# wolfi/NeuroSync_Trainer_Lite

Hardware: AMD Instinct MI355X
Metric: train frames/sec (audio->blendshape) 228M cfg (higher is better)
Workload: dtype bf16

## Files before the change

neurosync_trainer_lite_amd/csrc/gemm4.h:

```cpp
#pragma once
#include "common.h"
#include <type_traits>

namespace g4 {

constexpr int NT = 256;
constexpr int TILE = 256;
constexpr int BK = 64;
constexpr int OPS = 32768;
constexpr int SMEM = 4 * OPS;
constexpr int ROPE_LDS = 32768;
constexpr int GROUP_MAX = 16;

enum { EM_BF16 = 1, EM_RELU_DROP = 2, EM_ROPE = 3, EM_DRELU = 4, EM_F32 = 5 };

struct Params {
  const char* A; int64_t lda;
  const char* B; int64_t ldb;
  char* C; int64_t ldc;
  int M, N, K;
  float alpha;
  const float* bias;
  float inv_keep; uint32_t thresh; uint64_t seed;
  const float* rope_cos; const float* rope_sin; int rope_T, rope_dim, rope_cols;
  float* colsum_part;
  uint64_t* relu_mask;
  float* sq_part;
  const float* a_scale;
  const float* b_scale;
  int rope_bf16;
  uint32_t a_bytes, b_bytes;
  int tiles_m, tiles_n;
};

struct StreamK {
  float* slab;
  unsigned* cnt;
  uint32_t slab_bytes;
  int dp_tiles;
  int units;
};

struct GroupParams {
  Params g[GROUP_MAX];
  int tile_end[GROUP_MAX];
  int n;
  StreamK sk;
};
static_assert(sizeof(GroupParams) <= 4096, "kernel arguments");

typedef int i32x4_t __attribute__((ext_vector_type(4)));
typedef int i32x2_t __attribute__((ext_vector_type(2)));
typedef __attribute__((address_space(3))) void lds_void_t;

NSTL_DEV uint32_t lds_addr(const char* p) { return (uint32_t)(uintptr_t)(const __attribute__((address_space(3))) char*)p; }

#define G4_VMCNT(n) asm volatile("s_waitcnt vmcnt(" #n ")" ::: "memory")
#define G4_SB() __builtin_amdgcn_sched_barrier(0)
#define G4_LGKM0()                                      \
  do {                                                  \
    asm volatile("s_waitcnt lgkmcnt(0)" ::: "memory"); \
    G4_SB();                                            \
  } while (0)

NSTL_DEV void dma16(__amdgpu_buffer_rsrc_t r, char* lds, uint32_t voff, uint32_t soff) {
  __builtin_amdgcn_raw_ptr_buffer_load_lds(r, (lds_void_t*)lds, 16, voff, soff, 0, 0);
}

constexpr int SIDE_W = 2048;
constexpr int SIDE_LDS = 4 * SIDE_W;

template <bool KMAJ>
NSTL_DEV void dma_lane_offsets(uint32_t (&vo)[8], int64_t ld, int wave, int lane) {
#pragma unroll
  for (int s = 0; s < 8; ++s) {
    const int q = wave * 8 + s;
    if (KMAJ) {
      const int row = 8 * q + (lane >> 3), pc = lane & 7;
      const int lc = pc ^ ((row >> 1) & 7);
      vo[s] = (uint32_t)(((int64_t)row * ld + lc * 8) * 2);
    } else {
      const int row = 2 * q + (lane >> 5), pc = lane & 31;
// ... 118 lines not shown
                        char* bdst, uint32_t sa, uint32_t sb) {
  if constexpr (I < 64) {
    if constexpr (!(DBG & 8)) {
      if constexpr (Z) mma16z(acc[I >> 3][I & 7], cb[I & 7], ca[I >> 3]);
      else mma16(acc[I >> 3][I & 7], cb[I & 7], ca[I >> 3]);
    }
    G4_SB();
    if constexpr (RD && !(DBG & 2))
      rd_after<AK, BKM, RSOA, RSOB, RH, I, 0, (DBG & 256) ? 56 : (DBG & 512) ? 32 : (DBG & 1024) ? 24 : 46>(na, nb, ra,
                                                                                                       rb);
    if constexpr ((DMAM == 2 || DMAM == 3) && !(DBG & 1) && (I & 7) == ((DBG & 2048) ? 6 : 2)) {
      constexpr int q = I >> 3;
      if constexpr (DMAM == 2) dma16(d.ra, adst + q * 1024, d.va[q], d.ta + sa);
      else dma16(d.rb, bdst + q * 1024, d.vb[q], d.tb + sb);
      G4_SB();
    }
    constexpr bool DMA_HERE = (DBG & 16)    ? I < 16
                              : (DBG & 32)  ? (I < 32 && (I & 1) == 0)
                              : (DBG & 64)  ? (I >= 32 && (I & 1) == 0)
                              : (DBG & 128) ? (I >= 47 && I < 63)
                                            : (I & 3) == 2;
    if constexpr (DMAM == 1 && !(DBG & 1) && DMA_HERE) {
      constexpr int q = (DBG & 16)    ? I
                        : (DBG & 32)  ? I >> 1
                        : (DBG & 64)  ? (I - 32) >> 1
                        : (DBG & 128) ? I - 47
                                      : I >> 2;
      if constexpr (q < 8) dma16(d.ra, adst + q * 1024, d.va[q], d.ta + sa);
      else dma16(d.rb, bdst + (q - 8) * 1024, d.vb[q - 8], d.tb + sb);
      G4_SB();
    }
    half_step<AK, BKM, RD, RSOA, RSOB, RH, DMAM, DBG, Z, I + 1>(acc, ca, cb, na, nb, ra, rb, d, adst, bdst, sa, sb);
  }
}

NSTL_DEV void tile_coords(int id, int nt_m, int nt_n, int& m0, int& n0) {
  constexpr int GROUP_M = 4;
  const int per_group = GROUP_M * nt_n;
  const int first_m = (id / per_group) * GROUP_M;
  const int gm = min(nt_m - first_m, GROUP_M);
  const int in_g = id % per_group;
  m0 = (first_m + in_g % gm) * TILE;
  n0 = (in_g / gm) * TILE;
}

typedef float f32x2_t __attribute__((ext_vector_type(2)));
typedef __bf16 bf16x2_t __attribute__((ext_vector_type(2)));
NSTL_DEV uint32_t pack_bf16x2(float lo, float hi) {
  return __builtin_bit_cast(uint32_t, __builtin_convertvector((f32x2_t){lo, hi}, bf16x2_t));
}
NSTL_DEV float bf16_lo(uint32_t w) { return __uint_as_float(w << 16); }
NSTL_DEV float bf16_hi(uint32_t w) { return __uint_as_float(w & 0xFFFF0000u); }
NSTL_DEV uint32_t asr31(uint32_t x) {
  uint32_t r;
  asm("v_ashrrev_i32 %0, 31, %1" : "=v"(r) : "v"(x));
  return r;
}
NSTL_DEV uint32_t min1(uint32_t x) {
  uint32_t r;
  asm("v_min_u32 %0, 1, %1" : "=v"(r) : "v"(x));
  return r;
}
NSTL_DEV uint32_t keep_lo_mask(uint32_t h, uint32_t thresh) { return asr31(thresh - 1u - (h & 0xFFFFu)); }
NSTL_DEV uint32_t keep_hi_mask(uint32_t h, uint32_t thresh) { return asr31(thresh - 1u - (h >> 16)); }
NSTL_DEV float and_mask(float x, uint32_t m) { return __uint_as_float(__float_as_uint(x) & m); }
NSTL_DEV uint32_t pos_bits2(uint32_t w) {
// ... 58 lines not shown
  float r0, r1, r2, r3;
  if constexpr (ZW == 2) {
    asm volatile(
        "v_accvgpr_read_b32 %0, %4\n\t"
        "v_accvgpr_read_b32 %1, %5\n\t"
        "v_accvgpr_read_b32 %2, %6\n\t"
        "v_accvgpr_read_b32 %3, %7"
        : "=&v"(r0), "=&v"(r1), "=&v"(r2), "=&v"(r3)
        : "a"(x[0]), "a"(x[1]), "a"(x[2]), "a"(x[3]));
    asm volatile("v_mfma_f32_16x16x16_bf16 %0, %1, %1, 0" : "+a"(x) : "v"(z));
  } else if constexpr (ZW == 1) {
    asm volatile(
        "v_accvgpr_read_b32 %0, %4\n\t"
        "v_accvgpr_read_b32 %1, %5\n\t"
        "v_accvgpr_read_b32 %2, %6\n\t"
        "v_accvgpr_read_b32 %3, %7\n\t"
        "v_accvgpr_write_b32 %4, 0\n\t"
        "v_accvgpr_write_b32 %5, 0\n\t"
        "v_accvgpr_write_b32 %6, 0\n\t"
        "v_accvgpr_write_b32 %7, 0"
        : "=&v"(r0), "=&v"(r1), "=&v"(r2), "=&v"(r3), "+a"(x[0]), "+a"(x[1]), "+a"(x[2]), "+a"(x[3]));
  } else {
    asm volatile(
        "v_accvgpr_read_b32 %0, %4\n\t"
        "v_accvgpr_read_b32 %1, %5\n\t"
        "v_accvgpr_read_b32 %2, %6\n\t"
        "v_accvgpr_read_b32 %3, %7"
        : "=&v"(r0), "=&v"(r1), "=&v"(r2), "=&v"(r3)
        : "a"(x[0]), "a"(x[1]), "a"(x[2]), "a"(x[3]));
  }
  return (f32x4){r0, r1, r2, r3};
}

NSTL_DEV f32x4 rd_acc_keep(const f32x4& x) {
  float r0, r1, r2, r3;
  asm volatile(
      "v_accvgpr_read_b32 %0, %4\n\t"
      "v_accvgpr_read_b32 %1, %5\n\t"
      "v_accvgpr_read_b32 %2, %6\n\t"
      "v_accvgpr_read_b32 %3, %7"
      : "=&v"(r0), "=&v"(r1), "=&v"(r2), "=&v"(r3)
      : "a"(x[0]), "a"(x[1]), "a"(x[2]), "a"(x[3]));
  return (f32x4){r0, r1, r2, r3};
}
NSTL_DEV void add_acc(f32x4& x, const f32x4 y) {
  float t0, t1, t2, t3;
  asm volatile(
      "v_accvgpr_read_b32 %0, %4\n\t"
      "v_accvgpr_read_b32 %1, %5\n\t"
      "v_accvgpr_read_b32 %2, %6\n\t"
      "v_accvgpr_read_b32 %3, %7\n\t"
      "v_add_f32 %0, %0, %8\n\t"
      "v_add_f32 %1, %1, %9\n\t"
      "v_add_f32 %2, %2, %10\n\t"
      "v_add_f32 %3, %3, %11\n\t"
      "v_accvgpr_write_b32 %4, %0\n\t"
      "v_accvgpr_write_b32 %5, %1\n\t"
      "v_accvgpr_write_b32 %6, %2\n\t"
      "v_accvgpr_write_b32 %7, %3"
      : "=&v"(t0), "=&v"(t1), "=&v"(t2), "=&v"(t3), "+a"(x[0]), "+a"(x[1]), "+a"(x[2]), "+a"(x[3])
      : "v"(y[0]), "v"(y[1]), "v"(y[2]), "v"(y[3]));
}

struct Seg {
  int t, ks, ke;
};
struct Walker {
  int t_dp, G, dp_tiles, U;
  int rank;
  int pos, end;
  NSTL_DEV void init(const GroupParams& gp, int T, int w, int G_, bool sk) {
    G = G_;
    t_dp = w;
    rank = w;
    if (sk) {
      dp_tiles = gp.sk.dp_tiles;
      U = gp.sk.units;
      if (G % 8 == 0) rank = xcd_remap(w, G);
      const int I = (T - dp_tiles) * U;
      pos = rank * I / G;
      end = (rank + 1) * I / G;
    } else {
      dp_tiles = T;
      U = 1;
      pos = end = 0;
    }
  }
  NSTL_DEV bool next(Seg& s) {
    if (t_dp < dp_tiles) {
      s.t = t_dp;
      s.ks = 0;
      s.ke = -1;
      t_dp += G;
      return true;
    }
    if (pos >= end) return false;
    s.t = dp_tiles + pos / U;
    s.ks = pos % U;
    s.ke = s.ks + end - pos < U ? s.ks + end - pos : U;
    pos += s.ke - s.ks;
    return true;
  }
};

NSTL_DEV bool sk_handoff(const StreamK& sk, f32x4 (&acc)[8][8], const Seg& s, int w, int wave, int lane) {
  const bool part = !(s.ke < 0 || (s.ks == 0 && s.ke == sk.units));
  const bool tail = s.ks > 0;
  const uint32_t mine = (uint32_t)(tail ? 2 * w : 2 * w + 1), other = (uint32_t)(tail ? 2 * w - 1 : 2 * w + 2);
  const __amdgpu_buffer_rsrc_t r =
      __builtin_amdgcn_make_buffer_rsrc((void*)sk.slab, 0, part ? (int)sk.slab_bytes : 0, 0x00020000);
// ... 265 lines not shown
          uint32_t lo = (uint32_t)w, hi = (uint32_t)(w >> 32);
          lo |= (uint32_t)__builtin_amdgcn_mov_dpp((int)lo, 0x128, 0xF, 0xF, false);
          hi |= (uint32_t)__builtin_amdgcn_mov_dpp((int)hi, 0x128, 0xF, 0xF, false);
          const auto slo = __builtin_amdgcn_permlane16_swap(lo, lo, false, false);
          const auto shi = __builtin_amdgcn_permlane16_swap(hi, hi, false, false);
          lo = slo[0] | slo[1];
          hi = shi[0] | shi[1];
          if (fin && c < 8 && odd == 0)
            p.relu_mask[mask_word(p.N, row0 + 64 * hb + c, col0 + 16 * b + 4 * g)] = ((uint64_t)hi << 32) | lo;
        }
    }
    if (EM == EM_DRELU && p.colsum_part != nullptr) {
#pragma unroll
      for (int b = 0; b < 8; ++b)
#pragma unroll
        for (int e = 0; e < 4; ++e) {
          float x = csum[b][e];
          x += NSTL_DPP(x, 0xB1);
          x += NSTL_DPP(x, 0x4E);
          x += NSTL_DPP(x, 0x141);
          x += NSTL_DPP(x, 0x140);
          csum[b][e] = x;
        }
      if (fin && c == 0) {
        float* dst = p.colsum_part + (int64_t)(row0 >> 7) * p.N + col0 + 4 * g;
#pragma unroll
        for (int b = 0; b < 8; ++b) *(f32x4*)(dst + 16 * b) = (f32x4){csum[b][0], csum[b][1], csum[b][2], csum[b][3]};
      }
    }
  }
}

template <bool AK, bool BKM, int EM, bool GROUPED, int DBG = 0, bool SK = false, int R3 = 0>
__global__ __launch_bounds__(NT, 1) void gemm4_kernel(const GroupParams gp) {
  constexpr bool A3 = R3 == 1, B3 = R3 == 2;
  static_assert(!(R3 && EM == EM_ROPE), "the 3 + 2 ring fills the LDS: no room for the RoPE table");
  constexpr bool SIDE = !R3 && (EM == EM_BF16 || (EM == EM_RELU_DROP && BKM) || EM == EM_DRELU) && !(DBG & 16384);
  constexpr int SMEM_ALL = R3 ? 5 * OPS : SMEM + (EM == EM_ROPE ? ROPE_LDS : 0) + (SIDE ? SIDE_LDS : 0);
  constexpr int B_BASE = A3 ? 3 * OPS : 2 * OPS;
  constexpr bool ZC = !BKM && !SK;
  __shared__ __attribute__((aligned(16))) char smem[SMEM_ALL];
  const int tid = threadIdx.x, lane = tid & 63;
  const int wave = __builtin_amdgcn_readfirstlane(tid >> 6);
  const int wm = wave >> 1, wn = wave & 1;
  const int T = gp.tile_end[gp.n - 1];
  const int G = gridDim.x;
  Walker wk;
  wk.init(gp, T, blockIdx.x, G, SK);
  Seg sg;
  if (!wk.next(sg)) return;
  const uint32_t smem_u32 = lds_addr(smem);
  char* const adst0 = smem + wave * 8 * 1024;
  char* const bdst0 = smem + B_BASE + wave * 8 * 1024;
  const char* rope_lds = smem + SMEM;
  char* const side = smem + SMEM + wave * SIDE_W;
  if constexpr (EM == EM_ROPE) {
    const Params& p0 = gp.g[0];
    const int half = p0.rope_dim >> 1, chunks = p0.rope_dim >> 2, swz = rope_swz(p0.rope_dim);
    for (int i = tid; i < p0.rope_T * chunks; i += NT) {
      const int tt = i / chunks, k = i - tt * chunks;
      const float2 cs = *(const float2*)(p0.rope_cos + tt * half + 2 * k);
      const float2 sn = *(const float2*)(p0.rope_sin + tt * half + 2 * k);
      *(f32x4*)(smem + SMEM + rope_off(tt, k, p0.rope_dim * 4, swz)) = (f32x4){cs.x, sn.x, cs.y, sn.y};
    }
    __syncthreads();
  }

  const int ndp_all = SK ? gp.sk.dp_tiles : T;
  auto locate = [&](int tt, int& prob, int& m0, int& n0, int& lt) {
    const int gt = tt < ndp_all ? xcd_remap(tt, ndp_all) : tt;
    prob = 0;
    if (GROUPED)
      while (prob + 1 < gp.n && gt >= gp.tile_end[prob]) ++prob;
    const int first = prob ? gp.tile_end[prob - 1] : 0;
    const Params& q = gp.g[prob];
    lt = gt - first;
    tile_coords(lt, q.tiles_m, q.tiles_n, m0, n0);
  };
  int prob, m0, n0, lt;
  locate(sg.t, prob, m0, n0, lt);
  Dma d;
  dma_lanes<AK, BKM>(d, gp.g[prob], wave, lane);
  dma_tile<AK, BKM>(d, gp.g[prob], m0, n0, sg.ks);
  RdAddr<AK> ra;
  RdAddr<BKM> rb;
  rd_addr<AK>(ra, smem_u32, wm * 128, lane);
  rd_addr<BKM>(rb, smem_u32 + B_BASE, wn * 128, lane);

  f32x4 acc[8][8];
#pragma unroll
  for (int a = 0; a < 8; ++a)
#pragma unroll
    for (int b = 0; b < 8; ++b) acc[a][b] = (f32x4){0.f, 0.f, 0.f, 0.f};
  bf16x8 f0a[8], f0b[8], f1a[8], f1b[8];
#pragma unroll
  for (int s = 0; s < 2; ++s) {
#pragma unroll
    for (int q = 0; q < 8; ++q) dma16(d.ra, adst0 + s * OPS + q * 1024, d.va[q], d.ta + (uint32_t)s * d.a_kb);
#pragma unroll
    for (int q = 0; q < 8; ++q) dma16(d.rb, bdst0 + s * OPS + q * 1024, d.vb[q], d.tb + (uint32_t)s * d.b_kb);
  }
  G4_VMCNT(0);
  __builtin_amdgcn_s_barrier();
  G4_SB();
  rd_all<AK, BKM, 0>(f0a, f0b, ra, rb);
  G4_LGKM0();

  int s3_cur = 0;
  auto move3 = [&](int from, int to) {
    const uint32_t delta = (uint32_t)((to - from) * OPS);
    if constexpr (A3) {
      if constexpr (AK) {
#pragma unroll
        for (int h = 0; h < 2; ++h) ra.k[h] += delta;
      } else {
#pragma unroll
        for (int j = 0; j < 8; ++j) ra.t[j] += delta;
      }
    } else if constexpr (B3) {
      if constexpr (BKM) {
#pragma unroll
        for (int h = 0; h < 2; ++h) rb.k[h] += delta;
      } else {
#pragma unroll
        for (int j = 0; j < 8; ++j) rb.t[j] += delta;
      }
    }
  };

  auto step = [&](auto slot_c, auto waitn_c, uint32_t dma_stage, const Dma& dd) {
    constexpr int S = decltype(slot_c)::value;
    constexpr int WAITN = decltype(waitn_c)::value;
    if constexpr (R3 && WAITN != 0 && !(DBG & 4096)) {
      const int s3_dma = s3_cur == 0 ? 2 : s3_cur - 1;
      const int s3_next = s3_cur == 2 ? 0 : s3_cur + 1;
      const uint32_t oa = dma_stage * dd.a_kb, ob = dma_stage * dd.b_kb;
      half_step<AK, BKM, true, A3 ? 0 : S * OPS, B3 ? 0 : S * OPS, 1, 0, DBG, ZC>(acc, f0a, f0b, f1a, f1b, ra, rb,
                                                                               dd, adst0, bdst0, 0, 0);
      G4_LGKM0();
      if constexpr (WAITN == 32) G4_VMCNT(32);
      else G4_VMCNT(63);
      __builtin_amdgcn_s_barrier();
      G4_SB();
      move3(s3_cur, s3_next);
      half_step<AK, BKM, true, A3 ? 0 : (1 - S) * OPS, B3 ? 0 : (1 - S) * OPS, 0, 1, DBG>(
          acc, f1a, f1b, f0a, f0b, ra, rb, dd, adst0 + (A3 ? s3_dma : S) * OPS, bdst0 + (B3 ? s3_dma : S) * OPS, oa,
          ob);
      G4_LGKM0();
      s3_cur = s3_next;
    } else if constexpr (R3) {
      const int s3_dma = s3_cur == 0 ? 2 : s3_cur - 1;
      const int s3_next = s3_cur == 2 ? 0 : s3_cur + 1;
      const uint32_t oa = dma_stage * dd.a_kb, ob = dma_stage * dd.b_kb;
      half_step<AK, BKM, true, A3 ? 0 : S * OPS, B3 ? 0 : S * OPS, 1, A3 ? 2 : 3, DBG, ZC && WAITN != 0>(
          acc, f0a, f0b, f1a, f1b, ra, rb, dd, adst0 + s3_dma * OPS, bdst0 + s3_dma * OPS, oa, ob);
      G4_LGKM0();
      if constexpr (WAITN == 0) G4_VMCNT(8);
      else if constexpr (WAITN == 32) G4_VMCNT(40);
      else G4_VMCNT(63);
      __builtin_amdgcn_s_barrier();
      G4_SB();
      move3(s3_cur, s3_next);
      half_step<AK, BKM, true, A3 ? 0 : (1 - S) * OPS, B3 ? 0 : (1 - S) * OPS, 0, A3 ? 3 : 2, DBG>(
          acc, f1a, f1b, f0a, f0b, ra, rb, dd, adst0 + S * OPS, bdst0 + S * OPS, oa, ob);
      G4_LGKM0();
      s3_cur = s3_next;
    } else {
      half_step<AK, BKM, true, S * OPS, S * OPS, 1, 0, DBG, ZC && WAITN != 0>(acc, f0a, f0b, f1a, f1b, ra, rb, dd,
                                                                              adst0, bdst0, 0, 0);
      G4_LGKM0();
      if constexpr (WAITN == 0) G4_VMCNT(0);
      else if constexpr (WAITN == 32) G4_VMCNT(32);
      else G4_VMCNT(63);
      __builtin_amdgcn_s_barrier();
      G4_SB();
      half_step<AK, BKM, true, (1 - S) * OPS, (1 - S) * OPS, 0, 1, DBG>(acc, f1a, f1b, f0a, f0b, ra, rb, dd,
                                                                      adst0 + S * OPS, bdst0 + S * OPS,
                                                                      dma_stage * dd.a_kb, dma_stage * dd.b_kb);
      G4_LGKM0();
    }
  };
  using S0 = std::integral_constant<int, 0>;
  using S1 = std::integral_constant<int, 1>;
  using W0 = std::integral_constant<int, 0>;
  using WE = std::integral_constant<int, EM == EM_F32 ? 63 : 32>;

  for (;;) {
    const Params& p = gp.g[prob];
    const int nk = sg.ke < 0 ? p.K / BK : 4 * (sg.ke - sg.ks);
    Seg ns;
    const bool has_next = wk.next(ns);
    if (!has_next) ns = sg;
    int nprob = prob, nm0 = m0, nn0 = n0, nlt = lt;
    if (has_next) locate(ns.t, nprob, nm0, nn0, nlt);
    if constexpr (SIDE) side_dma<EM>(p, side, m0 + wm * 128, n0 + wn * 128, lane);
    step(S0{}, WE{}, 2u, d);
    for (int kt = 1; kt < nk; kt += 2) {
      step(S1{}, W0{}, (uint32_t)(kt + 2 < nk ? kt + 2 : kt + 2 - nk), d);
      if (kt + 1 < nk) {
        if (kt + 1 == nk - 2) {
          if (GROUPED && nprob != prob) dma_lanes<AK, BKM>(d, gp.g[nprob], wave, lane);
          dma_tile<AK, BKM>(d, gp.g[nprob], nm0, nn0, ns.ks, has_next || (DBG & 32768));
        }
        step(S0{}, W0{}, (uint32_t)(kt + 3 < nk ? kt + 3 : kt + 3 - nk), d);
      }
    }
    bool fin = true;
    if constexpr (SK) fin = sk_handoff(gp.sk, acc, sg, wk.rank, wave, lane);
    epilogue<EM, false, (DBG & 8192) ? 1 : 0, ZC ? 0 : (SK ? 1 : 2), SIDE>(p, acc, m0 + wm * 128, n0 + wn * 128, lane,
                                                                        wave, lt, rope_lds, fin, side);
    if (!has_next) break;
    sg = ns;
    prob = nprob;
    m0 = nm0;
    n0 = nn0;
    lt = nlt;
  }
  G4_VMCNT(0);
}

constexpr int F8_BK = 128;

typedef int i32x8_t __attribute__((ext_vector_type(8)));

NSTL_DEV void mma_f8(f32x4& acc, const i32x8_t& w, const i32x8_t& x) {
  acc = __builtin_amdgcn_mfma_scale_f32_16x16x128_f8f6f4(w, x, acc, 0, 0, 0, 0x7f7f7f7f, 0, 0x7f7f7f7f);
}
NSTL_DEV void mma_f8z(f32x4& acc, const i32x8_t& w, const i32x8_t& x) {
  acc = __builtin_amdgcn_mfma_scale_f32_16x16x128_f8f6f4(w, x, (f32x4){0.f, 0.f, 0.f, 0.f}, 0, 0, 0, 0x7f7f7f7f, 0,
                                                          0x7f7f7f7f);
}

NSTL_DEV void dma_lane_offsets_f8(uint32_t (&vo)[8], int64_t ld, int wave, int lane) {
#pragma unroll
  for (int s = 0; s < 8; ++s) {
    const int q = wave * 8 + s;
    const int row = 8 * q + (lane >> 3), pc = lane & 7;
    const int lc = pc ^ ((row >> 1) & 7);
    vo[s] = (uint32_t)((int64_t)row * ld + lc * 16);
  }
}
NSTL_DEV void dma_tile_f8(Dma& d, const Params& p, int m0, int n0, bool live = true) {
  d.ra = __builtin_amdgcn_make_buffer_rsrc((void*)p.A, 0, live ? (int)p.a_bytes : 0, 0x00020000);
  d.rb = __builtin_amdgcn_make_buffer_rsrc((void*)p.B, 0, live ? (int)p.b_bytes : 0, 0x00020000);
  d.a_kb = F8_BK;
  d.b_kb = F8_BK;
  d.ta = __builtin_amdgcn_readfirstlane((uint32_t)(m0 * p.lda));
  d.tb = __builtin_amdgcn_readfirstlane((uint32_t)(n0 * p.ldb));
}

struct RdAddrF8 {
// ... 23 lines not shown
      G4_SB();
    }
    if constexpr (!(DBG & 8)) {
      if constexpr (Z) mma_f8z(acc[4 * (H ? 1 : 0) + a][b], cb[b], ca[a]);
      else mma_f8(acc[4 * (H ? 1 : 0) + a][b], cb[b], ca[a]);
    }
    G4_SB();
    if constexpr (!(DBG & 2)) {
      if constexpr (H == 0 && (I == 1 || I == 6 || I == 11 || I == 16)) {
        constexpr int r = I == 1 ? 0 : I == 6 ? 1 : I == 11 ? 2 : 3;
        rd_f8<SO + (4 + r) * 2048>(na[r], ra);
        G4_SB();
      }
      if constexpr (H == 1 && (I & 7) == 0) {
        rd_f8<SO + (I >> 3) * 2048>(na[I >> 3], ra);
        G4_SB();
      }
      if constexpr (H == 1 && a == 3) {
        rd_f8<SO + b * 2048>(cb[b], rb);
        G4_SB();
      }
    }
    if constexpr (H >= 1 && !(DBG & 1) && (I & 1) == 1) {
      constexpr int q = I >> 1;
      if constexpr (q < 8) dma16(d.ra, adst + q * 1024, d.va[q], d.ta + sa);
      else dma16(d.rb, bdst + (q - 8) * 1024, d.vb[q - 8], d.tb + sb);
      G4_SB();
    }
    half_step_f8<H, SO, DBG, Z, I + 1>(acc, ca, cb, na, ra, rb, d, adst, bdst, sa, sb);
  }
}

template <int EM, int DBG = 0>
__global__ __launch_bounds__(NT, 1) void gemm4f8_kernel(const GroupParams gp) {
  constexpr bool SIDE = EM != EM_ROPE && EM != EM_F32 && !(DBG & 16384);
  __shared__ __attribute__((aligned(16))) char smem[SMEM + (EM == EM_ROPE ? ROPE_LDS : 0) + (SIDE ? 4 * SIDE_W_SC : 0)];
  const int tid = threadIdx.x, lane = tid & 63;
  const int wave = __builtin_amdgcn_readfirstlane(tid >> 6);
  const int wm = wave >> 1, wn = wave & 1;
  const int T = gp.tile_end[0];
  const int G = gridDim.x;
  const Params& p = gp.g[0];
  Walker wk;
  wk.init(gp, T, blockIdx.x, G, false);
  Seg sg;
  if (!wk.next(sg)) return;
  const uint32_t smem_u32 = lds_addr(smem);
  char* const adst0 = smem + wave * 8 * 1024;
  char* const bdst0 = smem + 2 * OPS + wave * 8 * 1024;
  const char* rope_lds = smem + SMEM;
  char* const side = smem + SMEM + wave * SIDE_W_SC;
  if constexpr (EM == EM_ROPE) {
    const int half = p.rope_dim >> 1, chunks = p.rope_dim >> 2, swz = rope_swz(p.rope_dim);
    for (int i = tid; i < p.rope_T * chunks; i += NT) {
      const int tt = i / chunks, k = i - tt * chunks;
      const float2 cs = *(const float2*)(p.rope_cos + tt * half + 2 * k);
      const float2 sn = *(const float2*)(p.rope_sin + tt * half + 2 * k);
      if (p.rope_bf16) {
        *(uint2*)(smem + SMEM + rope_off8(tt, k, p.rope_dim * 2, swz)) =
            make_uint2(pack_bf16x2(cs.x, sn.x), pack_bf16x2(cs.y, sn.y));
      } else {
        *(f32x4*)(smem + SMEM + rope_off(tt, k, p.rope_dim * 4, swz)) = (f32x4){cs.x, sn.x, cs.y, sn.y};
      }
    }
    __syncthreads();
  }
  int m0, n0;
  tile_coords(xcd_remap(sg.t, T), p.tiles_m, p.tiles_n, m0, n0);
  int lt = 0;
  Dma d;
  dma_lane_offsets_f8(d.va, p.lda, wave, lane);
  dma_lane_offsets_f8(d.vb, p.ldb, wave, lane);
  dma_tile_f8(d, p, m0, n0);
  RdAddrF8 ra, rb;
  rd_addr_f8(ra, smem_u32, wm * 128, lane);
  rd_addr_f8(rb, smem_u32 + 2 * OPS, wn * 128, lane);

// ... 80 lines not shown
```

neurosync_trainer_lite_amd/csrc/gemm4.hip:

```cpp
#include <stdlib.h>
#include <string.h>

#include <map>
#include <mutex>
#include <vector>

#include "../../include/nstl.h"
#include "common.h"
#include "gemm4.h"
#include "status.h"

namespace {

int gemm4_env() {
  const char* e = getenv("NSTL_GEMM4");
  return e ? atoi(e) : 1;
}

int sk_env() {
  const char* e = getenv("NSTL_GEMM4_SK");
  return e ? atoi(e) : 0;
}

struct SkSpace {
  float* slab = nullptr;
  unsigned* cnt = nullptr;
  int G = 0;
};
constexpr size_t SK_SPACES = 4;
bool sk_space(hipStream_t st, int G, g4::StreamK& sk) {
  static std::mutex mu;
  static std::map<std::pair<int, hipStream_t>, SkSpace> spaces;
  static std::vector<SkSpace> retired;
  const int dev = nstl::stream_device(st);
  std::lock_guard<std::mutex> lk(mu);
  if (spaces.find({dev, st}) == spaces.end() && spaces.size() >= SK_SPACES) return false;
  SkSpace& s = spaces[{dev, st}];
  if (s.G < G) {
    nstl::DeviceGuard on(dev);
    hipStreamCaptureStatus cs = hipStreamCaptureStatusNone;
    if (hipStreamIsCapturing(st, &cs) != hipSuccess || cs != hipStreamCaptureStatusNone) return false;
    if (s.slab) retired.push_back(s);
    s = SkSpace();
    if (hipMalloc((void**)&s.slab, (size_t)2 * G * 262144) != hipSuccess) return false;
    if (hipMalloc((void**)&s.cnt, (size_t)8 * G * sizeof(unsigned)) != hipSuccess) return false;
    if (hipMemset(s.cnt, 0, (size_t)8 * G * sizeof(unsigned)) != hipSuccess) return false;
    s.G = G;
  }
  sk.slab = s.slab;
  sk.cnt = s.cnt;
  sk.slab_bytes = (uint32_t)((size_t)2 * G * 262144);
  return true;
}

void plan_sk(g4::GroupParams& gp, int G, hipStream_t st) {
  memset(&gp.sk, 0, sizeof(gp.sk));
  const int T = gp.tile_end[gp.n - 1];
  const int mode = sk_env();
  if (T < G || !mode || (T % G == 0 && mode != 2)) return;
  const int K = gp.g[0].K;
  for (int i = 0; i < gp.n; ++i)
    if (gp.g[i].K != K) return;
  if (K % (4 * g4::BK)) return;
  g4::StreamK sk;
  if (!sk_space(st, G, sk)) {
    (void)hipGetLastError();
    return;
  }
  sk.dp_tiles = (T / G - 1) * G;
  sk.units = K / (4 * g4::BK);
  gp.sk = sk;
}

int g4_mode(const nstl_gemm_args* a) {
  if (a->dtype != NSTL_BF16 || a->split_k > 1 || a->beta != 0.f || (a->sq_part != nullptr && a->c_dtype != NSTL_F32))
    return 0;
  const bool bf_out = a->c_dtype == NSTL_BF16;
  if (a->colsum_part != nullptr && a->epilogue != NSTL_EPI_DRELU_DROP) return 0;
  if (a->relu_mask != nullptr && a->epilogue != NSTL_EPI_BIAS_RELU_DROP && a->epilogue != NSTL_EPI_DRELU_DROP)
    return 0;
  switch (a->epilogue) {
    case NSTL_EPI_NONE:
      return bf_out ? g4::EM_BF16 : g4::EM_F32;
    case NSTL_EPI_BIAS:
      return bf_out ? g4::EM_BF16 : 0;
    case NSTL_EPI_BIAS_RELU_DROP:
      return bf_out && (a->N & 1) == 0 ? g4::EM_RELU_DROP : 0;
    case NSTL_EPI_BIAS_ROPE:
      return bf_out && a->b_kmajor && a->rope_dim % 4 == 0 && a->rope_cols % 16 == 0 &&
// ... 19 lines not shown
  return ae < (1ll << 31) && be < (1ll << 31) && ce < (1ll << 31);
}

void fill(g4::Params& q, const nstl_gemm_args* a) {
  memset(&q, 0, sizeof(q));
  q.A = (const char*)a->A; q.lda = a->lda;
  q.B = (const char*)a->B; q.ldb = a->ldb;
  q.C = (char*)a->C; q.ldc = a->ldc;
  q.M = a->M; q.N = a->N; q.K = a->K;
  q.alpha = a->alpha;
  q.bias = a->bias;
  q.thresh = nstl_drop_thresh(a->p_drop);
  q.inv_keep = 1.0f / (1.0f - a->p_drop);
  q.seed = a->seed;
  q.rope_cos = a->rope_cos; q.rope_sin = a->rope_sin;
  q.rope_T = a->rope_T; q.rope_dim = a->rope_dim; q.rope_cols = a->rope_cols;
  q.colsum_part = a->colsum_part;
  q.relu_mask = a->relu_mask;
  q.sq_part = a->sq_part;
  q.a_bytes = (uint32_t)(a->a_kmajor ? ((int64_t)(a->M - 1) * a->lda + a->K) * 2 : ((int64_t)(a->K - 1) * a->lda + a->M) * 2);
  q.b_bytes = (uint32_t)(a->b_kmajor ? ((int64_t)(a->N - 1) * a->ldb + a->K) * 2 : ((int64_t)(a->K - 1) * a->ldb + a->N) * 2);
  q.tiles_m = a->M / g4::TILE;
  q.tiles_n = a->N / g4::TILE;
}

int r3_env() {
  const char* e = getenv("NSTL_GEMM4_R3");
  return e ? atoi(e) : 1;
}

template <bool AK, bool BKM, bool GROUPED, bool SK, int R3>
void launch_em(int em, dim3 grid, hipStream_t st, const g4::GroupParams& gp) {
  const dim3 block(g4::NT);
  switch (em) {
    case g4::EM_BF16: hipLaunchKernelGGL((g4::gemm4_kernel<AK, BKM, g4::EM_BF16, GROUPED, 0, SK, R3>), grid, block, 0, st, gp); break;
    case g4::EM_RELU_DROP:
      hipLaunchKernelGGL((g4::gemm4_kernel<AK, BKM, g4::EM_RELU_DROP, GROUPED, 0, SK, R3>), grid, block, 0, st, gp);
      break;
    case g4::EM_ROPE:
      if constexpr (BKM && !R3) hipLaunchKernelGGL((g4::gemm4_kernel<AK, BKM, g4::EM_ROPE, GROUPED, 0, SK>), grid, block, 0, st, gp);
      break;
    case g4::EM_DRELU: hipLaunchKernelGGL((g4::gemm4_kernel<AK, BKM, g4::EM_DRELU, GROUPED, 0, SK, R3>), grid, block, 0, st, gp); break;
    default: hipLaunchKernelGGL((g4::gemm4_kernel<AK, BKM, g4::EM_F32, GROUPED, 0, SK, R3>), grid, block, 0, st, gp); break;
  }
}

template <bool SK, int R3>
int launch_sk(int em, bool ak, bool bk, bool grouped, dim3 grid, hipStream_t st, const g4::GroupParams& gp) {
  if (ak && bk) {
    if (grouped) {
      if (em != g4::EM_ROPE || SK || R3) return 0;
      hipLaunchKernelGGL((g4::gemm4_kernel<true, true, g4::EM_ROPE, true, 0, false, 0>), grid, dim3(g4::NT), 0, st, gp);
      return 1;
    }
    launch_em<true, true, false, SK, R3>(em, grid, st, gp);
  } else if (ak && !bk) {
    if (grouped) return 0;
    launch_em<true, false, false, SK, R3>(em, grid, st, gp);
  } else {
    if (em != g4::EM_F32) return 0;
    if (grouped) hipLaunchKernelGGL((g4::gemm4_kernel<false, false, g4::EM_F32, true, 0, SK, R3>), grid, dim3(g4::NT), 0, st, gp);
    else hipLaunchKernelGGL((g4::gemm4_kernel<false, false, g4::EM_F32, false, 0, SK, R3>), grid, dim3(g4::NT), 0, st, gp);
  }
  return 1;
}

int launch(int em, bool ak, bool bk, bool grouped, int G, hipStream_t st, g4::GroupParams& gp) {
  const int tiles = gp.tile_end[gp.n - 1];
  const dim3 grid(tiles < G ? tiles : G);
  plan_sk(gp, G, st);
  if (!gp.sk.slab) {
    int kmin = gp.g[0].K;
    for (int i = 1; i < gp.n; ++i) kmin = gp.g[i].K < kmin ? gp.g[i].K : kmin;
    if (em != g4::EM_ROPE && kmin >= 2048 && r3_env()) return launch_sk<false, 1>(em, ak, bk, grouped, grid, st, gp);
    return launch_sk<false, 0>(em, ak, bk, grouped, grid, st, gp);
  }
  if (!launch_sk<true, 0>(em, ak, bk, grouped, grid, st, gp)) return 0;
  nstl::count(NSTL_K_GEMM4_SK);
  return 1;
}

int g4f8_mode(const nstl_gemm_args* a) {
  if (a->dtype != NSTL_FP8 || a->split_k > 1 || a->beta != 0.f || !a->a_kmajor || !a->b_kmajor) return 0;
  if (!a->a_scale || !a->b_scale || a->sq_part) return 0;
  const bool bf_out = a->c_dtype == NSTL_BF16;
  if (a->colsum_part != nullptr && a->epilogue != NSTL_EPI_DRELU_DROP) return 0;
  if (a->relu_mask != nullptr && a->epilogue != NSTL_EPI_BIAS_RELU_DROP && a->epilogue != NSTL_EPI_DRELU_DROP)
    return 0;
  switch (a->epilogue) {
    case NSTL_EPI_NONE: return bf_out ? g4::EM_BF16 : 0;
    case NSTL_EPI_BIAS: return bf_out ? g4::EM_BF16 : 0;
    case NSTL_EPI_BIAS_RELU_DROP: return bf_out && (a->N & 1) == 0 ? g4::EM_RELU_DROP : 0;
    case NSTL_EPI_BIAS_ROPE:
      return bf_out && a->rope_dim % 4 == 0 && a->rope_cols % 16 == 0 &&
                     (int64_t)a->rope_T * a->rope_dim * 2 <= g4::ROPE_LDS
// ... 8 lines not shown
  if (a->M % g4::TILE || a->N % g4::TILE || a->K % (2 * g4::F8_BK) || a->K < 4 * g4::F8_BK) return false;
  if (((uintptr_t)a->A | (uintptr_t)a->B | (uintptr_t)a->C) % 16) return false;
  if (a->lda % 16 || a->ldb % 16) return false;
  if (a->ldc % (a->c_dtype == NSTL_F32 ? 4 : 8)) return false;
  const int64_t ae = (int64_t)(a->M - 1) * a->lda + a->K, be = (int64_t)(a->N - 1) * a->ldb + a->K;
  const int64_t ce = a->c_dtype == NSTL_F32 ? (int64_t)a->M * a->ldc * 4 : 0;
  return ae < (1ll << 31) && be < (1ll << 31) && ce < (1ll << 31);
}

}

namespace nstl {

int gemm4_f8(const nstl_gemm_args* a, hipStream_t st, int* handled) {
  *handled = 0;
  const char* e = getenv("NSTL_GEMM4_F8");
  if ((e && atoi(e) == 0) || !gemm4_env() || !g4f8_shape_ok(a)) return 0;
  const int em = g4f8_mode(a);
  if (!em) return 0;
  const int G = nstl::stream_cus(st);
  if (G <= 0) return 0;
  g4::GroupParams gp;
  memset(&gp, 0, sizeof(gp));
  g4::Params& q = gp.g[0];
  fill(q, a);
  q.a_bytes = (uint32_t)((int64_t)(a->M - 1) * a->lda + a->K);
  q.b_bytes = (uint32_t)((int64_t)(a->N - 1) * a->ldb + a->K);
  q.a_scale = a->a_scale;
  q.b_scale = a->b_scale;
  q.rope_bf16 = em == g4::EM_ROPE && (int64_t)a->rope_T * a->rope_dim * 4 > g4::ROPE_LDS;
  gp.n = 1;
  gp.tile_end[0] = q.tiles_m * q.tiles_n;
  const dim3 grid(gp.tile_end[0] < G ? gp.tile_end[0] : G), block(g4::NT);
  switch (em) {
    case g4::EM_BF16: hipLaunchKernelGGL((g4::gemm4f8_kernel<g4::EM_BF16>), grid, block, 0, st, gp); break;
    case g4::EM_RELU_DROP: hipLaunchKernelGGL((g4::gemm4f8_kernel<g4::EM_RELU_DROP>), grid, block, 0, st, gp); break;
    case g4::EM_ROPE: hipLaunchKernelGGL((g4::gemm4f8_kernel<g4::EM_ROPE>), grid, block, 0, st, gp); break;
    default: hipLaunchKernelGGL((g4::gemm4f8_kernel<g4::EM_DRELU>), grid, block, 0, st, gp); break;
  }
  NSTL_LAUNCH_CHECK("nstl_gemm (fp8, 4-wave persistent)");
  nstl::count(NSTL_K_GEMM_FP8);
  nstl::count(NSTL_K_GEMM4F8);
  if (em == g4::EM_ROPE) nstl::count(NSTL_K_GEMM_FP8_ROPE);
  nstl::count(NSTL_K_GEMM4_TILES, gp.tile_end[0]);
  *handled = 1;
  return 0;
}

int gemm4(const nstl_gemm_args* a, hipStream_t st, int* handled) {
  *handled = 0;
  if (!gemm4_env() || !g4_shape_ok(a)) return 0;
  const int em = g4_mode(a);
  if (!em) return 0;
  if (!a->a_kmajor && em != g4::EM_F32) return 0;
  const int G = nstl::stream_cus(st);
  if (G <= 0) return 0;
  g4::GroupParams gp;
  memset(&gp, 0, sizeof(gp));
  fill(gp.g[0], a);
  gp.n = 1;
  gp.tile_end[0] = gp.g[0].tiles_m * gp.g[0].tiles_n;
  if (!launch(em, a->a_kmajor, a->b_kmajor, false, G, st, gp)) return 0;
  NSTL_LAUNCH_CHECK("nstl_gemm (4-wave persistent)");
  nstl::count(NSTL_K_GEMM4);
  nstl::count(NSTL_K_GEMM4_TILES, gp.tile_end[0]);
  *handled = 1;
  return 0;
}

int gemm4_grouped(const nstl_gemm_args* args, int n, hipStream_t st, int* handled) {
  *handled = 0;
// ... 30 lines not shown
```

Before: 652,600.

## Shrink GEMM kernel args and overlap first-tile prefetch with setup

Non-grouped launches now pass a compact one-problem argument struct instead of the full 16-entry GroupParams, which cuts kernel-argument size and preload cost. The first two K-stage DMAs are issued before the RoPE table fill and accumulator zeroing, so that setup overlaps the loads. The first step waits only for the first stage (vmcnt 16) rather than draining all loads, and a runtime-branching wait helper applies a stricter wait on the first tile only. It also adds optional timestamp instrumentation behind a debug flag and drops the memset of sk in plan_sk, which depends on callers zeroing gp beforehand.

Result: no change. 658,100, median of 6 (+0.8%).

```diff
diff --git a/neurosync_trainer_lite_amd/csrc/gemm4.h b/neurosync_trainer_lite_amd/csrc/gemm4.h
--- a/neurosync_trainer_lite_amd/csrc/gemm4.h
+++ b/neurosync_trainer_lite_amd/csrc/gemm4.h
@@ -31,6 +31,7 @@
   int rope_bf16;
   uint32_t a_bytes, b_bytes;
   int tiles_m, tiles_n;
+  unsigned long long* stamps;
 };
 
 struct StreamK {
@@ -48,6 +49,32 @@
   StreamK sk;
 };
 static_assert(sizeof(GroupParams) <= 4096, "kernel arguments");
+
+struct OneParams {
+  Params g[1];
+  int tile_end[1];
+  static constexpr int n = 1;
+};
+struct OneParamsSK {
+  Params g[1];
+  int tile_end[1];
+  static constexpr int n = 1;
+  StreamK sk;
+};
+template <bool GROUPED, bool SK>
+using KArgs = std::conditional_t<GROUPED, GroupParams, std::conditional_t<SK, OneParamsSK, OneParams>>;
+template <bool GROUPED, bool SK>
+inline KArgs<GROUPED, SK> kargs(const GroupParams& gp) {
+  if constexpr (GROUPED) {
+    return gp;
+  } else {
+    KArgs<GROUPED, SK> k{};
+    k.g[0] = gp.g[0];
+    k.tile_end[0] = gp.tile_end[0];
+    if constexpr (SK) k.sk = gp.sk;
+    return k;
+  }
+}
 
 typedef int i32x4_t __attribute__((ext_vector_type(4)));
 typedef int i32x2_t __attribute__((ext_vector_type(2)));
@@ -232,6 +259,36 @@
     }
     half_step<AK, BKM, RD, RSOA, RSOB, RH, DMAM, DBG, Z, I + 1>(acc, ca, cb, na, nb, ra, rb, d, adst, bdst, sa, sb);
   }
+}
+
+constexpr int STAMPS = 7;
+NSTL_DEV unsigned long long clock_stamp() {
+  unsigned long long t;
+  G4_SB();
+  asm volatile("s_memtime %0\n\ts_waitcnt lgkmcnt(0)" : "=s"(t)::"memory");
+  G4_SB();
+  return t;
+}
+NSTL_DEV unsigned long long real_stamp() {
+  unsigned long long t;
+  G4_SB();
+  asm volatile("s_memrealtime %0\n\ts_waitcnt lgkmcnt(0)" : "=s"(t)::"memory");
+  G4_SB();
+  return t;
+}
+
+template <int FIRST, int REST>
+NSTL_DEV void wait_step0(int first) {
+  static_assert(FIRST <= REST, "the first tile's wait is the stricter one");
+  asm volatile(
+      "s_cmp_eq_u32 %0, 0\n\t"
+      "s_cbranch_scc1 .Lg4_step0_%=\n\t"
+      "s_waitcnt vmcnt(%1)\n"
+      ".Lg4_step0_%=:\n\t"
+      "s_waitcnt vmcnt(%2)"
+      :
+      : "s"(first), "n"(FIRST), "n"(REST)
+      : "scc", "memory");
 }
 
 NSTL_DEV void tile_coords(int id, int nt_m, int nt_n, int& m0, int& n0) {
@@ -356,6 +413,15 @@
   return (f32x4){r0, r1, r2, r3};
 }
 
+NSTL_DEV void zero_acc(f32x4& x) {
+  asm volatile(
+      "v_accvgpr_write_b32 %0, 0\n\t"
+      "v_accvgpr_write_b32 %1, 0\n\t"
+      "v_accvgpr_write_b32 %2, 0\n\t"
+      "v_accvgpr_write_b32 %3, 0"
+      : "=a"(x[0]), "=a"(x[1]), "=a"(x[2]), "=a"(x[3]));
+}
+
 NSTL_DEV f32x4 rd_acc_keep(const f32x4& x) {
   float r0, r1, r2, r3;
   asm volatile(
@@ -393,13 +459,13 @@
   int t_dp, G, dp_tiles, U;
   int rank;
   int pos, end;
-  NSTL_DEV void init(const GroupParams& gp, int T, int w, int G_, bool sk) {
+  NSTL_DEV void init(const StreamK* sk, int T, int w, int G_) {
     G = G_;
     t_dp = w;
     rank = w;
     if (sk) {
-      dp_tiles = gp.sk.dp_tiles;
-      U = gp.sk.units;
+      dp_tiles = sk->dp_tiles;
+      U = sk->units;
       if (G % 8 == 0) rank = xcd_remap(w, G);
       const int I = (T - dp_tiles) * U;
       pos = rank * I / G;
@@ -731,7 +797,7 @@
 }
 
 template <bool AK, bool BKM, int EM, bool GROUPED, int DBG = 0, bool SK = false, int R3 = 0>
-__global__ __launch_bounds__(NT, 1) void gemm4_kernel(const GroupParams gp) {
+__global__ __launch_bounds__(NT, 1) void gemm4_kernel(const KArgs<GROUPED, SK> gp) {
   constexpr bool A3 = R3 == 1, B3 = R3 == 2;
   static_assert(!(R3 && EM == EM_ROPE), "the 3 + 2 ring fills the LDS: no room for the RoPE table");
   constexpr bool SIDE = !R3 && (EM == EM_BF16 || (EM == EM_RELU_DROP && BKM) || EM == EM_DRELU) && !(DBG & 16384);
@@ -739,13 +805,25 @@
   constexpr int B_BASE = A3 ? 3 * OPS : 2 * OPS;
   constexpr bool ZC = !BKM && !SK;
   __shared__ __attribute__((aligned(16))) char smem[SMEM_ALL];
+  constexpr bool STAMP = (DBG & 65536) != 0;
+  unsigned long long stamp[STAMPS] = {};
+  if constexpr (STAMP) {
+    stamp[5] = real_stamp();
+    stamp[0] = clock_stamp();
+  }
   const int tid = threadIdx.x, lane = tid & 63;
   const int wave = __builtin_amdgcn_readfirstlane(tid >> 6);
   const int wm = wave >> 1, wn = wave & 1;
   const int T = gp.tile_end[gp.n - 1];
   const int G = gridDim.x;
+  if constexpr (!GROUPED && !SK) {
+    const Params& q = gp.g[0];
+    asm volatile("" ::"s"(q.A), "s"(q.lda), "s"(q.B), "s"(q.ldb), "s"(q.a_bytes), "s"(q.b_bytes), "s"(q.tiles_m),
+                 "s"(q.tiles_n), "s"(T), "s"(G));
+  }
   Walker wk;
-  wk.init(gp, T, blockIdx.x, G, SK);
+  if constexpr (SK) wk.init(&gp.sk, T, blockIdx.x, G);
+  else wk.init(nullptr, T, blockIdx.x, G);
   Seg sg;
   if (!wk.next(sg)) return;
   const uint32_t smem_u32 = lds_addr(smem);
@@ -753,19 +831,9 @@
   char* const bdst0 = smem + B_BASE + wave * 8 * 1024;
   const char* rope_lds = smem + SMEM;
   char* const side = smem + SMEM + wave * SIDE_W;
-  if constexpr (EM == EM_ROPE) {
-    const Params& p0 = gp.g[0];
-    const int half = p0.rope_dim >> 1, chunks = p0.rope_dim >> 2, swz = rope_swz(p0.rope_dim);
-    for (int i = tid; i < p0.rope_T * chunks; i += NT) {
-      const int tt = i / chunks, k = i - tt * chunks;
-      const float2 cs = *(const float2*)(p0.rope_cos + tt * half + 2 * k);
-      const float2 sn = *(const float2*)(p0.rope_sin + tt * half + 2 * k);
-      *(f32x4*)(smem + SMEM + rope_off(tt, k, p0.rope_dim * 4, swz)) = (f32x4){cs.x, sn.x, cs.y, sn.y};
-    }
-    __syncthreads();
-  }
-
-  const int ndp_all = SK ? gp.sk.dp_tiles : T;
+
+  int ndp_all = T;
+  if constexpr (SK) ndp_all = gp.sk.dp_tiles;
   auto locate = [&](int tt, int& prob, int& m0, int& n0, int& lt) {
     const int gt = tt < ndp_all ? xcd_remap(tt, ndp_all) : tt;
     prob = 0;
@@ -781,6 +849,25 @@
   Dma d;
   dma_lanes<AK, BKM>(d, gp.g[prob], wave, lane);
   dma_tile<AK, BKM>(d, gp.g[prob], m0, n0, sg.ks);
+#pragma unroll
+  for (int s = 0; s < 2; ++s) {
+#pragma unroll
+    for (int q = 0; q < 8; ++q) dma16(d.ra, adst0 + s * OPS + q * 1024, d.va[q], d.ta + (uint32_t)s * d.a_kb);
+#pragma unroll
+    for (int q = 0; q < 8; ++q) dma16(d.rb, bdst0 + s * OPS + q * 1024, d.vb[q], d.tb + (uint32_t)s * d.b_kb);
+  }
+  G4_SB();
+  if constexpr (EM == EM_ROPE) {
+    const Params& p0 = gp.g[0];
+    const int half = p0.rope_dim >> 1, chunks = p0.rope_dim >> 2, swz = rope_swz(p0.rope_dim);
+    for (int i = tid; i < p0.rope_T * chunks; i += NT) {
+      const int tt = i / chunks, k = i - tt * chunks;
+      const float2 cs = *(const float2*)(p0.rope_cos + tt * half + 2 * k);
+      const float2 sn = *(const float2*)(p0.rope_sin + tt * half + 2 * k);
+      *(f32x4*)(smem + SMEM + rope_off(tt, k, p0.rope_dim * 4, swz)) = (f32x4){cs.x, sn.x, cs.y, sn.y};
+    }
+    G4_LGKM0();
+  }
   RdAddr<AK> ra;
   RdAddr<BKM> rb;
   rd_addr<AK>(ra, smem_u32, wm * 128, lane);
@@ -790,18 +877,16 @@
 #pragma unroll
   for (int a = 0; a < 8; ++a)
 #pragma unroll
-    for (int b = 0; b < 8; ++b) acc[a][b] = (f32x4){0.f, 0.f, 0.f, 0.f};
+    for (int b = 0; b < 8; ++b) {
+      if constexpr (ZC || SK) acc[a][b] = (f32x4){0.f, 0.f, 0.f, 0.f};
+      else zero_acc(acc[a][b]);
+    }
+  G4_SB();
   bf16x8 f0a[8], f0b[8], f1a[8], f1b[8];
-#pragma unroll
-  for (int s = 0; s < 2; ++s) {
-#pragma unroll
-    for (int q = 0; q < 8; ++q) dma16(d.ra, adst0 + s * OPS + q * 1024, d.va[q], d.ta + (uint32_t)s * d.a_kb);
-#pragma unroll
-    for (int q = 0; q < 8; ++q) dma16(d.rb, bdst0 + s * OPS + q * 1024, d.vb[q], d.tb + (uint32_t)s * d.b_kb);
-  }
-  G4_VMCNT(0);
+  G4_VMCNT(16);
   __builtin_amdgcn_s_barrier();
   G4_SB();
+  if constexpr (STAMP) stamp[1] = clock_stamp();
   rd_all<AK, BKM, 0>(f0a, f0b, ra, rb);
   G4_LGKM0();
 
@@ -827,6 +912,7 @@
     }
   };
 
+  int first = 1;
   auto step = [&](auto slot_c, auto waitn_c, uint32_t dma_stage, const Dma& dd) {
     constexpr int S = decltype(slot_c)::value;
     constexpr int WAITN = decltype(waitn_c)::value;
@@ -837,8 +923,7 @@
       half_step<AK, BKM, true, A3 ? 0 : S * OPS, B3 ? 0 : S * OPS, 1, 0, DBG, ZC>(acc, f0a, f0b, f1a, f1b, ra, rb,
                                                                                dd, adst0, bdst0, 0, 0);
       G4_LGKM0();
-      if constexpr (WAITN == 32) G4_VMCNT(32);
-      else G4_VMCNT(63);
+      wait_step0<0, WAITN>(first);
       __builtin_amdgcn_s_barrier();
       G4_SB();
       move3(s3_cur, s3_next);
@@ -855,8 +940,7 @@
           acc, f0a, f0b, f1a, f1b, ra, rb, dd, adst0 + s3_dma * OPS, bdst0 + s3_dma * OPS, oa, ob);
       G4_LGKM0();
       if constexpr (WAITN == 0) G4_VMCNT(8);
-      else if constexpr (WAITN == 32) G4_VMCNT(40);
-      else G4_VMCNT(63);
+      else wait_step0<8, WAITN == 32 ? 40 : 63>(first);
       __builtin_amdgcn_s_barrier();
       G4_SB();
       move3(s3_cur, s3_next);
@@ -869,8 +953,7 @@
                                                                               adst0, bdst0, 0, 0);
       G4_LGKM0();
       if constexpr (WAITN == 0) G4_VMCNT(0);
-      else if constexpr (WAITN == 32) G4_VMCNT(32);
-      else G4_VMCNT(63);
+      else wait_step0<0, WAITN>(first);
       __builtin_amdgcn_s_barrier();
       G4_SB();
       half_step<AK, BKM, true, (1 - S) * OPS, (1 - S) * OPS, 0, 1, DBG>(acc, f1a, f1b, f0a, f0b, ra, rb, dd,
@@ -895,6 +978,8 @@
     if constexpr (SIDE) side_dma<EM>(p, side, m0 + wm * 128, n0 + wn * 128, lane);
     step(S0{}, WE{}, 2u, d);
     for (int kt = 1; kt < nk; kt += 2) {
+      if constexpr (STAMP)
+        if (kt == nk - 1) stamp[2] = clock_stamp();
       step(S1{}, W0{}, (uint32_t)(kt + 2 < nk ? kt + 2 : kt + 2 - nk), d);
       if (kt + 1 < nk) {
         if (kt + 1 == nk - 2) {
@@ -909,13 +994,21 @@
     epilogue<EM, false, (DBG & 8192) ? 1 : 0, ZC ? 0 : (SK ? 1 : 2), SIDE>(p, acc, m0 + wm * 128, n0 + wn * 128, lane,
                                                                         wave, lt, rope_lds, fin, side);
     if (!has_next) break;
+    first = 0;
     sg = ns;
     prob = nprob;
     m0 = nm0;
     n0 = nn0;
     lt = nlt;
   }
+  if constexpr (STAMP) stamp[3] = clock_stamp();
   G4_VMCNT(0);
+  if constexpr (STAMP) {
+    stamp[4] = clock_stamp();
+    stamp[6] = real_stamp();
+    if (tid == 0)
+      for (int i = 0; i < STAMPS; ++i) gp.g[0].stamps[blockIdx.x * STAMPS + i] = stamp[i];
+  }
 }
 
 constexpr int F8_BK = 128;
@@ -1005,7 +1098,7 @@
 }
 
 template <int EM, int DBG = 0>
-__global__ __launch_bounds__(NT, 1) void gemm4f8_kernel(const GroupParams gp) {
+__global__ __launch_bounds__(NT, 1) void gemm4f8_kernel(const OneParams gp) {
   constexpr bool SIDE = EM != EM_ROPE && EM != EM_F32 && !(DBG & 16384);
   __shared__ __attribute__((aligned(16))) char smem[SMEM + (EM == EM_ROPE ? ROPE_LDS : 0) + (SIDE ? 4 * SIDE_W_SC : 0)];
   const int tid = threadIdx.x, lane = tid & 63;
@@ -1015,7 +1108,7 @@
   const int G = gridDim.x;
   const Params& p = gp.g[0];
   Walker wk;
-  wk.init(gp, T, blockIdx.x, G, false);
+  wk.init(nullptr, T, blockIdx.x, G);
   Seg sg;
   if (!wk.next(sg)) return;
   const uint32_t smem_u32 = lds_addr(smem);
diff --git a/neurosync_trainer_lite_amd/csrc/gemm4.hip b/neurosync_trainer_lite_amd/csrc/gemm4.hip
--- a/neurosync_trainer_lite_amd/csrc/gemm4.hip
+++ b/neurosync_trainer_lite_amd/csrc/gemm4.hip
@@ -54,7 +54,6 @@
 }
 
 void plan_sk(g4::GroupParams& gp, int G, hipStream_t st) {
-  memset(&gp.sk, 0, sizeof(gp.sk));
   const int T = gp.tile_end[gp.n - 1];
   const int mode = sk_env();
   if (T < G || !mode || (T % G == 0 && mode != 2)) return;
@@ -140,16 +139,17 @@
 template <bool AK, bool BKM, bool GROUPED, bool SK, int R3>
 void launch_em(int em, dim3 grid, hipStream_t st, const g4::GroupParams& gp) {
   const dim3 block(g4::NT);
+  const auto ka = g4::kargs<GROUPED, SK>(gp);
   switch (em) {
-    case g4::EM_BF16: hipLaunchKernelGGL((g4::gemm4_kernel<AK, BKM, g4::EM_BF16, GROUPED, 0, SK, R3>), grid, block, 0, st, gp); break;
+    case g4::EM_BF16: hipLaunchKernelGGL((g4::gemm4_kernel<AK, BKM, g4::EM_BF16, GROUPED, 0, SK, R3>), grid, block, 0, st, ka); break;
     case g4::EM_RELU_DROP:
-      hipLaunchKernelGGL((g4::gemm4_kernel<AK, BKM, g4::EM_RELU_DROP, GROUPED, 0, SK, R3>), grid, block, 0, st, gp);
+      hipLaunchKernelGGL((g4::gemm4_kernel<AK, BKM, g4::EM_RELU_DROP, GROUPED, 0, SK, R3>), grid, block, 0, st, ka);
       break;
     case g4::EM_ROPE:
-      if constexpr (BKM && !R3) hipLaunchKernelGGL((g4::gemm4_kernel<AK, BKM, g4::EM_ROPE, GROUPED, 0, SK>), grid, block, 0, st, gp);
+      if constexpr (BKM && !R3) hipLaunchKernelGGL((g4::gemm4_kernel<AK, BKM, g4::EM_ROPE, GROUPED, 0, SK>), grid, block, 0, st, ka);
       break;
-    case g4::EM_DRELU: hipLaunchKernelGGL((g4::gemm4_kernel<AK, BKM, g4::EM_DRELU, GROUPED, 0, SK, R3>), grid, block, 0, st, gp); break;
-    default: hipLaunchKernelGGL((g4::gemm4_kernel<AK, BKM, g4::EM_F32, GROUPED, 0, SK, R3>), grid, block, 0, st, gp); break;
+    case g4::EM_DRELU: hipLaunchKernelGGL((g4::gemm4_kernel<AK, BKM, g4::EM_DRELU, GROUPED, 0, SK, R3>), grid, block, 0, st, ka); break;
+    default: hipLaunchKernelGGL((g4::gemm4_kernel<AK, BKM, g4::EM_F32, GROUPED, 0, SK, R3>), grid, block, 0, st, ka); break;
   }
 }
 
@@ -168,7 +168,7 @@
   } else {
     if (em != g4::EM_F32) return 0;
     if (grouped) hipLaunchKernelGGL((g4::gemm4_kernel<false, false, g4::EM_F32, true, 0, SK, R3>), grid, dim3(g4::NT), 0, st, gp);
-    else hipLaunchKernelGGL((g4::gemm4_kernel<false, false, g4::EM_F32, false, 0, SK, R3>), grid, dim3(g4::NT), 0, st, gp);
+    else hipLaunchKernelGGL((g4::gemm4_kernel<false, false, g4::EM_F32, false, 0, SK, R3>), grid, dim3(g4::NT), 0, st, (g4::kargs<false, SK>(gp)));
   }
   return 1;
 }
@@ -243,11 +243,12 @@
   gp.n = 1;
   gp.tile_end[0] = q.tiles_m * q.tiles_n;
   const dim3 grid(gp.tile_end[0] < G ? gp.tile_end[0] : G), block(g4::NT);
+  const g4::OneParams ka = g4::kargs<false, false>(gp);
   switch (em) {
-    case g4::EM_BF16: hipLaunchKernelGGL((g4::gemm4f8_kernel<g4::EM_BF16>), grid, block, 0, st, gp); break;
-    case g4::EM_RELU_DROP: hipLaunchKernelGGL((g4::gemm4f8_kernel<g4::EM_RELU_DROP>), grid, block, 0, st, gp); break;
-    case g4::EM_ROPE: hipLaunchKernelGGL((g4::gemm4f8_kernel<g4::EM_ROPE>), grid, block, 0, st, gp); break;
-    default: hipLaunchKernelGGL((g4::gemm4f8_kernel<g4::EM_DRELU>), grid, block, 0, st, gp); break;
+    case g4::EM_BF16: hipLaunchKernelGGL((g4::gemm4f8_kernel<g4::EM_BF16>), grid, block, 0, st, ka); break;
+    case g4::EM_RELU_DROP: hipLaunchKernelGGL((g4::gemm4f8_kernel<g4::EM_RELU_DROP>), grid, block, 0, st, ka); break;
+    case g4::EM_ROPE: hipLaunchKernelGGL((g4::gemm4f8_kernel<g4::EM_ROPE>), grid, block, 0, st, ka); break;
+    default: hipLaunchKernelGGL((g4::gemm4f8_kernel<g4::EM_DRELU>), grid, block, 0, st, ka); break;
   }
   NSTL_LAUNCH_CHECK("nstl_gemm (fp8, 4-wave persistent)");
   nstl::count(NSTL_K_GEMM_FP8);
```
